# JacksonCampolattaro/spectrogram-rs

Hardware: AMD Instinct MI355X
Metric: STFT frames/sec (4096-pt, hop 256) (higher is better)
Workload: dtype f32

## Files before the change

spectrogram_rs_amd/csrc/stft4096_real.hip:

```cpp
#include <cmath>
#include <type_traits>

#include "stft4096_wg.hpp"

namespace sgx {

namespace wgr {

using wg::kBufComplex;
using wg::kLdsBytes;
using wg::kLdsBytesRender;
using wg::kM;
using wg::kS1;
using wg::kS2;
using wg::kW;
using wg::lds_barrier;
using wg::lds_read_alone;
using wg::lds_cfloat2;
using wg::lds_ptr;
using wg::pcm_rsrc;
using wg::u32x2;
using wg::u32x4;

typedef float f2v __attribute__((ext_vector_type(2)));
__device__ __forceinline__ float cl_fma(float a, float c, float u) { return fmaf(a, c, u); }
__device__ __forceinline__ f2v cl_fma(f2v a, float c, f2v u) { return __builtin_elementwise_fma(a, f2v{c, c}, u); }

#include "fft_codelets.inc"

using wg::Params;

__device__ __forceinline__ float2 cmulf(float2 a, float2 b)
{
    return make_float2(fmaf(a.x, b.x, -(a.y * b.y)), fmaf(a.x, b.y, a.y * b.x));
}

__device__ __forceinline__ __amdgpu_buffer_rsrc_t out_rsrc(char *base, long long byte, bool present)
{
    const uint32_t lo = __builtin_amdgcn_readfirstlane((uint32_t)byte);
    const uint32_t hi = __builtin_amdgcn_readfirstlane((uint32_t)((unsigned long long)byte >> 32));
    const int records = __builtin_amdgcn_readfirstlane(present ? 0x7fffffff : 0);
    return __builtin_amdgcn_make_buffer_rsrc(base + (long long)(((unsigned long long)hi << 32) | lo), 0, records, 0x00020000);
}

__device__ __forceinline__ void fft8_half_zero(const float (&zr)[4], const float (&zi)[4], float (&yr)[8], float (&yi)[8])
{
    constexpr float kH = 0.70710678118654752440f;
    auto fft4 = [](float a0r, float a0i, float a1r, float a1i, float a2r, float a2i, float a3r, float a3i, float *outr, float *outi) {
        const float s0r = a0r + a2r, s0i = a0i + a2i, s1r = a0r - a2r, s1i = a0i - a2i;
        const float s2r = a1r + a3r, s2i = a1i + a3i, s3r = a1r - a3r, s3i = a1i - a3i;
        outr[0] = s0r + s2r; outi[0] = s0i + s2i;
        outr[4] = s0r - s2r; outi[4] = s0i - s2i;
        outr[2] = s1r + s3i; outi[2] = s1i - s3r;
        outr[6] = s1r - s3i; outi[6] = s1i + s3r;
    };
    fft4(zr[0], zi[0], zr[1], zi[1], zr[2], zi[2], zr[3], zi[3], yr, yi);
    const float y1r = (zr[1] + zi[1]) * kH, y1i = (zi[1] - zr[1]) * kH;
    const float y3r = (zi[3] - zr[3]) * kH, y3i = -(zr[3] + zi[3]) * kH;
    fft4(zr[0], zi[0], y1r, y1i, zi[2], -zr[2], y3r, y3i, yr + 1, yi + 1);
}

constexpr int kRowsF32 = 0, kRowsF16 = 1, kPixels = 2;
constexpr int kBands = 3;
constexpr int kPeak = 5;
constexpr int kRowsC64 = 4;

#ifndef SGX_K1R_INTERLEAVE
#define SGX_K1R_INTERLEAVE 1
#endif
#ifndef SGX_SAMPLE_EARLY
#define SGX_SAMPLE_EARLY 1
#endif
#ifndef SGX_ADDTID_R
#define SGX_ADDTID_R 1
#endif
constexpr int kPlaneIm = 4480;
constexpr int kBufComplexTR = kPlaneIm;
static_assert(kBufComplexTR >= kBufComplex && 16 * 280 <= kPlaneIm, "the planes hold both images");
constexpr size_t kLdsBytesR = (size_t)(kBufComplexTR + 256) * sizeof(float2);
constexpr size_t kLdsBytesRenderR = kLdsBytesR + 256 * sizeof(uint2);
static_assert(4 * kLdsBytesRenderR <= 160 * 1024, "four workgroups per CU");
template <int STRIDE>
__device__ __forceinline__ void addtid_rows(float2 a, float2 b, uint32_t m0_wave, int ra, int rb)
{
    asm volatile("s_mov_b32 m0, %4\n\t"
                 "s_nop 0\n\t"
                 "ds_write_addtid_b32 %0 offset:%5\n\t"
                 "ds_write_addtid_b32 %1 offset:%6\n\t"
                 "ds_write_addtid_b32 %2 offset:%7\n\t"
                 "ds_write_addtid_b32 %3 offset:%8"
                 :
                 : "v"(a.x), "v"(a.y), "v"(b.x), "v"(b.y), "s"(m0_wave), "i"(4 * STRIDE * ra), "i"(4 * STRIDE * ra + 4 * kPlaneIm), "i"(4 * STRIDE * rb), "i"(4 * STRIDE * rb + 4 * kPlaneIm)
                 : "memory");
}
__device__ __forceinline__ void read_planes(const float4 *rd4, float (&xr)[16], float (&xi)[16])
{
#pragma unroll
    for (int c = 0; c < 4; ++c) {
        const float4 r = rd4[c], i = rd4[c + kPlaneIm / 4];
        xr[4 * c] = r.x; xr[4 * c + 1] = r.y; xr[4 * c + 2] = r.z; xr[4 * c + 3] = r.w;
        xi[4 * c] = i.x; xi[4 * c + 1] = i.y; xi[4 * c + 2] = i.z; xi[4 * c + 3] = i.w;
    }
}
__device__ __forceinline__ float lane_xor8(float v) { return __int_as_float(__builtin_amdgcn_mov_dpp(__float_as_int(v), 0x128, 0xf, 0xf, true)); }

#if SGX_STAMPS
__device__ unsigned long long g_phase_cycles_r[24];
#define SGX_STAMP(i) { const unsigned long long now_ = __builtin_readcyclecounter(); st_acc[i] += now_ - st_last; st_last = now_; }
#else
#define SGX_STAMP(i)
#endif

template <int MODE, int PIX, bool SLIDE>
__global__ void __launch_bounds__(256, 4) stft4096_real_kernel(Params p)
{
    extern __shared__ __attribute__((aligned(16))) unsigned char smem_raw[];
    float2 *buf = reinterpret_cast<float2 *>(smem_raw);
    constexpr bool TR = SLIDE && SGX_ADDTID_R;
    float2 *tw2 = buf + (TR ? kBufComplexTR : kBufComplex);
    uint2 *pal = reinterpret_cast<uint2 *>(tw2 + 256);
    constexpr bool F16 = MODE == kRowsF16;
    constexpr bool C64 = MODE == kRowsC64;
    constexpr bool FUSED = MODE == kPixels || MODE == kBands || MODE == kPeak;

    const int tid = threadIdx.x;
    const int t_p1 = TR ? (tid >> 4) + 16 * (tid & 15) : tid;
    float *plane = reinterpret_cast<float *>(smem_raw);
    const uint32_t m0_wave = __builtin_amdgcn_readfirstlane((uint32_t)(tid >> 6) * 272u);
    const float4 *rd4_1 = reinterpret_cast<const float4 *>(plane + 272 * (tid >> 4) + 68 * ((tid & 15) >> 2) + 16 * (tid & 3));
    const float4 *rd4_2 = reinterpret_cast<const float4 *>(plane + 280 * ((tid & 127) >> 3) + 68 * ((8 * (tid >> 7) + (tid & 7)) >> 2) + 16 * (tid & 3));
    tw2[tid] = p.tw2[tid];
    uint32_t row_words[4] = {0u, 0u, 0u, 0u};
    if (FUSED) {
        if (MODE == kPixels) pal[tid] = make_uint2(__float_as_uint(tid < 255 ? p.lut_thr[tid] : __builtin_nanf("")), *reinterpret_cast<const uint32_t *>(&p.lut_rgba[tid]));
#pragma unroll
        for (int i = 0; i < 4; ++i)
            if ((uint32_t)tid + 256u * i < p.R) row_words[i] = p.rows[tid + 256 * i];
    }

    float win[8];
#pragma unroll
    for (int a = 0; a < 4; ++a) {
        win[2 * a] = p.window[2 * t_p1 + 512 * a] * (1.0f / 2048.0f);
        win[2 * a + 1] = p.window[2 * t_p1 + 512 * a + 1] * (1.0f / 2048.0f);
    }
    float2 tw1[8];
#pragma unroll
    for (int q = 1; q < 8; ++q) tw1[q] = p.tw1[q * 256 + t_p1];
    const int F = tid >> 7, u = tid & 127;
    float2 twu[8];
#pragma unroll
    for (int q = 0; q < 8; ++q) twu[q] = p.twu[q * 128 + u];
    const int g2 = tid >> 4, t0_2 = tid & 15;
    const int cbase2 = (g2 >> 3) * 128 + (g2 & 7);
    __syncthreads();

    const unsigned long long job_begin = (unsigned long long)blockIdx.x * p.jobs_per_block;
    unsigned long long job_end = job_begin + p.jobs_per_block;
    if (job_end > p.n_jobs) job_end = p.n_jobs;
    if (job_begin >= job_end) return;

    auto samples_from = [&](unsigned long long first) {
        const unsigned long long left = first < p.stream_samples ? (p.stream_samples - first) * 4 : 0;
        const unsigned long long addr = (unsigned long long)(p.pcm + (first < p.stream_samples ? first : 0));
        const uint32_t lo = __builtin_amdgcn_readfirstlane((uint32_t)addr), hi = __builtin_amdgcn_readfirstlane((uint32_t)(addr >> 32));
        const int records = __builtin_amdgcn_readfirstlane((int)(left < 0x7fffffffull ? left : 0x7fffffffull));
        return __builtin_amdgcn_make_buffer_rsrc(reinterpret_cast<void *>(((unsigned long long)hi << 32) | lo), 0, records, 0x00020000);
    };
    auto columns_from = [&](unsigned long long col0) { return samples_from(2 * col0); };
    auto column = [&](__amdgpu_buffer_rsrc_t r, int byte_offset) {
        const u32x2 v = __builtin_amdgcn_raw_buffer_load_b64(r, t_p1 * 8, byte_offset, 0);
        return make_float2(__uint_as_float(v.x), __uint_as_float(v.y));
    };
    float2 R[8];
    float2 L;
    auto load_pair = [&](unsigned long long fa_) {
        const __amdgpu_buffer_rsrc_t r0 = samples_from(fa_ * p.H), r1 = samples_from((fa_ + 1) * p.H);
#pragma unroll
        for (int a = 0; a < 4; ++a) { R[2 * a] = column(r0, 2048 * a); R[2 * a + 1] = column(r1, 2048 * a); }
    };
    {
        const __amdgpu_buffer_rsrc_t r0 = columns_from(128 * (p.first_frame + 2 * job_begin));
        if (SLIDE) {
#pragma unroll
            for (int j = 0; j < 8; ++j) R[j] = column(r0, 1024 * j);
            L = column(r0, 9216);
        } else {
            load_pair(p.first_frame + 2 * job_begin);
            L = R[7];
        }
#pragma unroll
        for (int j = 0; j < 8; ++j) asm volatile("" ::"v"(R[j].x), "v"(R[j].y));
        asm volatile("" ::"v"(L.x), "v"(L.y));
#pragma unroll
        for (int q = 1; q < 8; ++q) asm volatile("" ::"v"(tw1[q].x), "v"(tw1[q].y));
#pragma unroll
        for (int q = 0; q < 8; ++q) asm volatile("" ::"v"(twu[q].x), "v"(twu[q].y), "v"(win[q]));
    }
    float2 *xch = buf + 2304;

    char *out = reinterpret_cast<char *>(p.mags);
    constexpr int kBin = C64 ? 16 : (F16 ? 4 : 8);
#if SGX_STAMPS
    unsigned long long st_acc[20] = {0, 0, 0, 0, 0, 0, 0, 0, 0, 0, 0, 0, 0, 0, 0, 0, 0, 0, 0, 0};
    unsigned long long st_last = __builtin_readcyclecounter();
#endif
    for (unsigned long long job = job_begin; job < job_end; ++job) {
        SGX_STAMP(19)
        const unsigned long long fa = p.first_frame + 2 * job;
        const unsigned long long la = 2 * job, lb = la + 1;
        const bool have_b = lb < p.n_frames;

        float yr[8], yi[8];
        {
            float zr[4], zi[4];
#pragma unroll
            for (int a = 0; a < 4; ++a) { zr[a] = R[2 * a].x * win[2 * a]; zi[a] = R[2 * a].y * win[2 * a + 1]; }
            fft8_half_zero(zr, zi, yr, yi);
        }
        float vr[8], vi[8];
        {
            float zr[4], zi[4];
#pragma unroll
            for (int a = 0; a < 4; ++a) { zr[a] = R[2 * a + 1].x * win[2 * a]; zi[a] = R[2 * a + 1].y * win[2 * a + 1]; }
            fft8_half_zero(zr, zi, vr, vi);
        }
        SGX_STAMP(0)
        lds_barrier();
        SGX_STAMP(1)
#pragma unroll
        for (int q = 0; q < 8; ++q) {
            const float2 ya = make_float2(yr[q], yi[q]), yb = make_float2(vr[q], vi[q]);
            if (TR) {
                addtid_rows<272>(q == 0 ? ya : cmulf(ya, tw1[q]), q == 0 ? yb : cmulf(yb, tw1[q]), m0_wave, q, 8 + q);
            } else {
                buf[q * kS1 + tid] = q == 0 ? ya : cmulf(ya, tw1[q]);
                buf[(8 + q) * kS1 + tid] = q == 0 ? yb : cmulf(yb, tw1[q]);
            }
        }
        __builtin_amdgcn_s_setprio(0);
        SGX_STAMP(2)
        lds_barrier();
        SGX_STAMP(3)

        float xr[16], xi[16];
        if (TR) {
            read_planes(rd4_1, xr, xi);
        } else {
#pragma unroll
            for (int t1 = 0; t1 < 16; ++t1) {
                const float2 v = buf[g2 * kS1 + t0_2 + 16 * t1];
                xr[t1] = v.x; xi[t1] = v.y;
            }
        }
        fft16(xr, xi);
        SGX_STAMP(4)
        lds_barrier();
        SGX_STAMP(5)
        if (TR) {
            lds_cfloat2 *tw2p = lds_ptr(tw2 + t0_2);
#pragma unroll
            for (int q2 = 0; q2 < 16; q2 += 2) {
                const int pa = FFT16_OUT[q2], pb = FFT16_OUT[q2 + 1];
                const float2 va = make_float2(xr[pa], xi[pa]), vb = make_float2(xr[pb], xi[pb]);
                addtid_rows<280>(q2 == 0 ? va : cmulf(va, lds_read_alone(tw2p, q2 * 16)), cmulf(vb, lds_read_alone(tw2p, (q2 + 1) * 16)), m0_wave, q2, q2 + 1);
            }
        } else {
#pragma unroll
            for (int q2 = 0; q2 < 16; ++q2) {
                const int pos = FFT16_OUT[q2];
                const float2 v = make_float2(xr[pos], xi[pos]);
                buf[t0_2 * kS2 + cbase2 + 8 * q2] = q2 == 0 ? v : cmulf(v, tw2[q2 * 16 + t0_2]);
            }
        }
        SGX_STAMP(6)
        lds_barrier();
        SGX_STAMP(7)

        if (TR) {
            read_planes(rd4_2, xr, xi);
        } else {
#pragma unroll
            for (int t0 = 0; t0 < 16; ++t0) {
                const float2 v = buf[t0 * kS2 + tid];
                xr[t0] = v.x; xi[t0] = v.y;
            }
        }
        fft16(xr, xi);

        float2 Ln = make_float2(0.0f, 0.0f);
        if (SLIDE && !FUSED) Ln = column(columns_from(128 * (fa + 2) + 1152), 0);
        if (!SLIDE) load_pair(fa + 2);

        if (FUSED) __builtin_amdgcn_s_setprio(1);
        else __builtin_amdgcn_s_setprio(3);
        SGX_STAMP(8)
        lds_barrier();
        SGX_STAMP(9)
#pragma unroll
        for (int j = 0; j < 8; ++j) {
            const int pos = FFT16_OUT[8 + j];
            buf[j * 256 + tid] = make_float2(xr[pos], xi[pos]);
        }
        if (SLIDE && !TR) {
            xch[tid].x = tid < 128 ? L.x : R[7].x;
            xch[tid].y = tid < 128 ? L.y : R[7].y;
        }
        SGX_STAMP(10)
        lds_barrier();
        SGX_STAMP(11)
        if (SLIDE) {
            const float2 Y = TR ? make_float2(lane_xor8((tid & 8) ? R[7].x : L.x), lane_xor8((tid & 8) ? R[7].y : L.y)) : xch[(tid + 128) & 255];
#pragma unroll
            for (int j = 0; j < 6; ++j) R[j] = R[j + 2];
            R[6] = Y;
            R[7] = L;
        }

        const int pcol = F * 128 + (u == 0 ? 256 : 128 - u);
        float m1[8], m2[8];
        constexpr bool kInterleave = (!FUSED && SLIDE && SGX_K1R_INTERLEAVE) || C64;
        const long long row = (long long)(F == 0 ? la : lb) * (long long)kM * kBin - kBin;
        const __amdgpu_buffer_rsrc_t r = out_rsrc(out, !FUSED ? row : 0, !FUSED && (F == 0 || have_b));
        const int l1 = kBin * u, l2 = kBin * (1152 - u);
        auto store_pair = [&](const int q3) {
            const float a = m1[q3], b = (q3 == 0 && u == 0) ? m1[0] : m2[q3];
            const int o1 = (q3 == 0 && u == 0) ? kBin * 1024 : l1;
            const int o2 = (q3 == 0 && u == 0) ? kBin * 128 : l2;
            const int s1 = kBin * 128 * q3, s2 = kBin * 128 * (7 - q3);
            if (F16) {
                const __half2 ha = __floats2half2_rn(a, a), hb = __floats2half2_rn(b, b);
                __builtin_amdgcn_raw_buffer_store_b32(*reinterpret_cast<const uint32_t *>(&ha), r, o1 + (s1 & 2047), s1 & ~2047, 0);
                __builtin_amdgcn_raw_buffer_store_b32(*reinterpret_cast<const uint32_t *>(&hb), r, o2 + (s2 & 2047), s2 & ~2047, 0);
            } else {
                __builtin_amdgcn_raw_buffer_store_b64(u32x2{__float_as_uint(a), __float_as_uint(a)}, r, o1 + (s1 & 2047), s1 & ~2047, 0);
                __builtin_amdgcn_raw_buffer_store_b64(u32x2{__float_as_uint(b), __float_as_uint(b)}, r, o2 + (s2 & 2047), s2 & ~2047, 0);
            }
        };
        float2 pvs[8];
        if (kInterleave) {
#pragma unroll
            for (int q3 = 0; q3 < 8; ++q3) pvs[q3] = buf[(7 - q3) * 256 + pcol];
        }
#pragma unroll
        for (int q3 = 0; q3 < 8; ++q3) {
            const int pos = FFT16_OUT[q3];
            float zr_ = xr[pos], zi_ = xi[pos];
            float2 pv = kInterleave ? pvs[q3] : buf[(7 - q3) * 256 + pcol];
            if (q3 == 0) {
                const float2 own = buf[F * 128];
                const int p8 = FFT16_OUT[8];
                zr_ = u == 0 ? xr[p8] : zr_; zi_ = u == 0 ? xi[p8] : zi_;
                pv.x = u == 0 ? own.x : pv.x; pv.y = u == 0 ? own.y : pv.y;
            }
            const float er = zr_ + pv.x, ei = zi_ - pv.y;
            const float orr = zi_ + pv.y, oi = pv.x - zr_;
            const float wr = fmaf(twu[q3].x, orr, -(twu[q3].y * oi)), wi = fmaf(twu[q3].x, oi, twu[q3].y * orr);
            const float ar = er + wr, ai = ei + wi, br = er - wr, bi = ei - wi;
            if constexpr (C64) {
                const bool self = q3 == 0 && u == 0;
                const float cr2 = self ? ar : br, ci2 = self ? ai : -bi;
                const int o1 = self ? kBin * 1024 : l1, o2 = self ? kBin * 128 : l2;
                const int s1 = kBin * 128 * q3, s2 = kBin * 128 * (7 - q3);
                __builtin_amdgcn_raw_buffer_store_b128(u32x4{__float_as_uint(ar), __float_as_uint(ai), __float_as_uint(ar), __float_as_uint(ai)}, r, o1 + s1, 0, 0);
                __builtin_amdgcn_raw_buffer_store_b128(u32x4{__float_as_uint(cr2), __float_as_uint(ci2), __float_as_uint(cr2), __float_as_uint(ci2)}, r, o2 + s2, 0, 0);
                __builtin_amdgcn_sched_barrier(0);
                continue;
            }
            m1[q3] = __builtin_amdgcn_sqrtf(fmaf(ar, ar, ai * ai));
            m2[q3] = __builtin_amdgcn_sqrtf(fmaf(br, br, bi * bi));
            if (kInterleave) {
                store_pair(q3);
                __builtin_amdgcn_sched_barrier(0);
            }
        }

        if (!FUSED) {
            if (!kInterleave) {
#pragma unroll
                for (int q3 = 0; q3 < 8; ++q3) store_pair(q3);
            }
        } else {
            float2 *mpair = buf;
            float2 *vbuf = mpair + wg::kColSlots;
            float *mcol = reinterpret_cast<float *>(buf) + F;
            lds_barrier();
            SGX_STAMP(13)
            constexpr bool kEarlyWords = SGX_SAMPLE_EARLY && PIX != wg::kPixGeneric;
            wg::SampleWords sw;
            const __amdgpu_buffer_rsrc_t rt_words = wg::pcm_rsrc(reinterpret_cast<const float *>(p.samples));
            int tid_w = tid;
            asm volatile("" : "+v"(tid_w));
#pragma unroll
            for (int q3 = 0; q3 < 8; ++q3) {
                const bool self = q3 == 0 && u == 0;
                const int k1 = self ? 1024 : u + 128 * q3, k2 = self ? 1024 : 2048 - u - 128 * q3;
                mcol[2 * k1] = m1[q3];
                mcol[2 * k2] = self ? m1[0] : m2[q3];
                if (q3 == 0 && u == 1) {
                    mcol[0] = m1[0];
                    mcol[2 * (kM + 1)] = mcol[2 * (kM + 2)] = m2[0];
                }
                if (kEarlyWords) {
                    sw.se[q3] = wg::sample_word(rt_words, p, (uint32_t)tid_w + 256u * q3);
                    __builtin_amdgcn_sched_barrier(0);
                }
            }
            if (kEarlyWords) sw.se[8] = wg::sample_word(rt_words, p, (uint32_t)tid_w + 2048u);
            static_assert(wg::kSampleSteps == 9 && wg::kSampleEarly == 9, "one word per column-write step and one behind them");
            SGX_STAMP(14)
            lds_barrier();
            SGX_STAMP(15)
            if (kEarlyWords) wg::sample_pass_with<PIX>(p, mpair, vbuf, tid, sw);
            else wg::sample_pass<PIX>(p, mpair, vbuf, tid);
            [[maybe_unused]] wg::PeakDst peak_a{}, peak_b{};
            [[maybe_unused]] wg::PeakOld<true> peak_old{};
            if constexpr (MODE == kPeak) {
                peak_a = wg::peak_dst(p, la);
                peak_b = have_b ? wg::peak_dst_next(p, peak_a, lb) : peak_a;
                peak_old = wg::peak_prefetch<true>(p, peak_a, tid);
            }
            if (SLIDE) L = column(columns_from(128 * (fa + 2) + 1152), 0);
            SGX_STAMP(16)
            lds_barrier();
            SGX_STAMP(17)
            __builtin_amdgcn_s_setprio(3);
            if constexpr (MODE == kPeak) {
                wg::row_pass_peak<true>(p, row_words, vbuf, peak_a, peak_b, peak_old, have_b, tid);
            } else if constexpr (MODE == kBands) {
                float2 *bands = reinterpret_cast<float2 *>(p.rgba);
                wg::row_pass_bands<true>(p, row_words, vbuf, bands + la * (size_t)p.R, bands + lb * (size_t)p.R, true, have_b, tid);
            } else {
                uchar4 *rgba = reinterpret_cast<uchar4 *>(p.rgba);
                wg::row_pass<true, PIX>(p, row_words, vbuf, rgba + la * (size_t)p.R, rgba + lb * (size_t)p.R, true, have_b, pal, tid);
            }
        }
        if (SLIDE && !FUSED) {
            asm volatile("" : "+v"(Ln.x), "+v"(Ln.y));
            L = Ln;
        }
        SGX_STAMP(18)
    }
#if SGX_STAMPS
    if ((tid & 63) == 0) {
#pragma unroll
        for (int i = 0; i < 20; ++i) atomicAdd(&g_phase_cycles_r[i], st_acc[i]);
        atomicAdd(&g_phase_cycles_r[20], (unsigned long long)(job_end - job_begin));
    }
#endif
}

struct RealTables {
    float2 *d_tw1 = nullptr, *d_tw2 = nullptr, *d_twu = nullptr;
};

}

#if SGX_STAMPS
extern "C" __attribute__((visibility("default"))) int sgx_debug_phase_cycles_r(unsigned long long *h_out, int reset)
{
    hipError_t e = hipMemcpyFromSymbol(h_out, HIP_SYMBOL(wgr::g_phase_cycles_r), sizeof(unsigned long long) * 24);
    if (e == hipSuccess && reset) {
        unsigned long long zero[24] = {0};
        e = hipMemcpyToSymbol(HIP_SYMBOL(wgr::g_phase_cycles_r), zero, sizeof(zero));
    }
    return e == hipSuccess ? 0 : -1;
}
#endif

hipError_t real4096_init(sgx_ctx *c, void **out)
{
    using namespace wgr;
    (void)c;
    auto *t = new RealTables();
    auto unit = [](unsigned long long e, unsigned long long n) {
        e %= n;
        if (e == 0) return make_float2(1.0f, 0.0f);
        if (4 * e == n) return make_float2(0.0f, -1.0f);
        if (2 * e == n) return make_float2(-1.0f, 0.0f);
        if (4 * e == 3 * n) return make_float2(0.0f, 1.0f);
        const double ang = -2.0 * M_PI * (double)e / (double)n;
        return make_float2((float)cos(ang), (float)sin(ang));
    };
    std::vector<float2> tw1(8 * 256), tw2(256), twu(8 * 128);
    for (int q = 0; q < 8; ++q)
        for (int tt = 0; tt < 256; ++tt) tw1[q * 256 + tt] = unit((unsigned long long)tt * q, 2048);
    for (int q = 0; q < 16; ++q)
        for (int t0 = 0; t0 < 16; ++t0) tw2[q * 16 + t0] = unit((unsigned long long)t0 * q, 256);
    for (int q3 = 0; q3 < 8; ++q3)
        for (int uu = 0; uu < 128; ++uu) twu[q3 * 128 + uu] = unit((unsigned long long)(uu + 128 * q3), 4096);
    twu[0] = unit(1024, 4096);
    auto up = [](float2 **dst, const std::vector<float2> &v) {
        hipError_t e = hipMalloc(reinterpret_cast<void **>(dst), v.size() * sizeof(float2));
        if (e == hipSuccess) e = hipMemcpy(*dst, v.data(), v.size() * sizeof(float2), hipMemcpyHostToDevice);
        return e;
    };
    hipError_t e = up(&t->d_tw1, tw1);
    if (e == hipSuccess) e = up(&t->d_tw2, tw2);
    if (e == hipSuccess) e = up(&t->d_twu, twu);
    if (e != hipSuccess) {
        real4096_destroy(t);
        return e;
    }
    *out = t;
    return hipSuccess;
}

void real4096_destroy(void *tables)
{
    auto *t = static_cast<wgr::RealTables *>(tables);
    if (!t) return;
    if (t->d_tw1) (void)hipFree(t->d_tw1);
    if (t->d_tw2) (void)hipFree(t->d_tw2);
    if (t->d_twu) (void)hipFree(t->d_twu);
    delete t;
}

bool real4096_serves(const sgx_ctx *c, const float *d_pcm, uint32_t channels)
{
    (void)d_pcm;
    return channels == 1 && c->d_real && c->W == (uint32_t)wgr::kW;
}

namespace wg {

hipError_t launch_real4096(const sgx_ctx *c, const void *real_tables, Params p, bool out_f16, bool render, bool bands, bool out_c64, bool peak)
{
    using namespace wgr;
    if (p.n_frames == 0) return hipSuccess;
    const auto *t = static_cast<const RealTables *>(real_tables);
    p.tw1 = t->d_tw1;
    p.tw2 = t->d_tw2;
    p.twu = t->d_twu;
    p.stream_samples = p.total_frames ? (p.total_frames - 1) * (unsigned long long)c->H + (unsigned long long)kW : 0;
    p.n_jobs = (p.n_frames + 1) / 2;
    unsigned long long blocks = (unsigned long long)c->n_cu * 4;
    unsigned long long per = (p.n_jobs + blocks - 1) / blocks;
    if (per < 1) per = 1;
    if (peak) {
        per = peak_align_run(per, 2, p.peak_group);
        p.peak_run = 2 * per;
    }
    blocks = (p.n_jobs + per - 1) / per;
    p.jobs_per_block = per;
    const dim3 grid((unsigned)blocks), block(256);
    auto launch = [&](auto slide_c) {
        constexpr bool S_ = decltype(slide_c)::value;
        constexpr size_t lds_rows = (S_ && SGX_ADDTID_R) ? kLdsBytesR : kLdsBytes, lds_render = (S_ && SGX_ADDTID_R) ? kLdsBytesRenderR : kLdsBytesRender;
        if (render && bands && peak) {
            if (p.interp == SGX_INTERP_COSINE) hipLaunchKernelGGL((stft4096_real_kernel<kPeak, kPixPeakCosine, S_>), grid, block, lds_rows, c->stream, p);
            else hipLaunchKernelGGL((stft4096_real_kernel<kPeak, kPixPeakCubic, S_>), grid, block, lds_rows, c->stream, p);
        } else if (render && bands) {
            if (p.interp == SGX_INTERP_COSINE) hipLaunchKernelGGL((stft4096_real_kernel<kBands, kPixBandsCosine, S_>), grid, block, lds_rows, c->stream, p);
            else hipLaunchKernelGGL((stft4096_real_kernel<kBands, kPixBandsCubic, S_>), grid, block, lds_rows, c->stream, p);
        } else if (render) {
            if (!p.seed_pm1) hipLaunchKernelGGL((stft4096_real_kernel<kPixels, kPixGeneric, S_>), grid, block, lds_render, c->stream, p);
            else if (p.interp == SGX_INTERP_COSINE) hipLaunchKernelGGL((stft4096_real_kernel<kPixels, kPixCosine, S_>), grid, block, lds_render, c->stream, p);
            else hipLaunchKernelGGL((stft4096_real_kernel<kPixels, kPixCubic, S_>), grid, block, lds_render, c->stream, p);
        } else if (out_c64) {
            hipLaunchKernelGGL((stft4096_real_kernel<kRowsC64, kPixNone, S_>), grid, block, lds_rows, c->stream, p);
        } else if (out_f16) {
            hipLaunchKernelGGL((stft4096_real_kernel<kRowsF16, kPixNone, S_>), grid, block, lds_rows, c->stream, p);
        } else {
            hipLaunchKernelGGL((stft4096_real_kernel<kRowsF32, kPixNone, S_>), grid, block, lds_rows, c->stream, p);
        }
    };
    if (c->H == 256) launch(std::true_type{});
    else launch(std::false_type{});
    const hipError_t e = hipGetLastError();
    return e == hipSuccess && peak ? launch_peak_combine(c, p, blocks) : e;
}

}

}
```

Baseline: 296.0 million.

## Defer row stores into next job and keep second-stage twiddles in registers

```diff
diff --git a/spectrogram_rs_amd/csrc/stft4096_real.hip b/spectrogram_rs_amd/csrc/stft4096_real.hip
--- a/spectrogram_rs_amd/csrc/stft4096_real.hip
+++ b/spectrogram_rs_amd/csrc/stft4096_real.hip
@@ -80,6 +80,25 @@
 constexpr size_t kLdsBytesR = (size_t)(kBufComplexTR + 256) * sizeof(float2);
 constexpr size_t kLdsBytesRenderR = kLdsBytesR + 256 * sizeof(uint2);
 static_assert(4 * kLdsBytesRenderR <= 160 * 1024, "four workgroups per CU");
+#ifndef SGX_K1R_HOLD
+#define SGX_K1R_HOLD 7
+#endif
+#ifndef SGX_K1R_PACE
+#define SGX_K1R_PACE 1
+#endif
+#ifndef SGX_K1R_PRIO
+#define SGX_K1R_PRIO 9
+#endif
+#ifndef SGX_K1R_PA
+#define SGX_K1R_PA 1
+#define SGX_K1R_PB 1
+#define SGX_K1R_PC 0
+#define SGX_K1R_PD 0
+#endif
+constexpr bool hold_level(int mode, bool slide, int bit) { return mode == 0  && slide && SGX_ADDTID_R && (SGX_K1R_HOLD & 1) && (SGX_K1R_HOLD & bit); }
+constexpr int kPartnerComplex = 8 * 256;
+constexpr size_t kLdsBytesHold = (SGX_K1R_HOLD & 4) ? (size_t)(kBufComplexTR + kPartnerComplex) * sizeof(float2) : kLdsBytesR;
+static_assert(3 * ((kLdsBytesHold + 1279) / 1280 * 1280) <= 160 * 1024, "three workgroups per CU (LDS is allocated in pieces of 1 280 B)");
 template <int STRIDE>
 __device__ __forceinline__ void addtid_rows(float2 a, float2 b, uint32_t m0_wave, int ra, int rb)
 {
@@ -112,7 +131,7 @@
 #endif
 
 template <int MODE, int PIX, bool SLIDE>
-__global__ void __launch_bounds__(256, 4) stft4096_real_kernel(Params p)
+__global__ void __launch_bounds__(256, hold_level(MODE, SLIDE, 1) ? 3 : 4) stft4096_real_kernel(Params p)
 {
     extern __shared__ __attribute__((aligned(16))) unsigned char smem_raw[];
     float2 *buf = reinterpret_cast<float2 *>(smem_raw);
@@ -122,6 +141,12 @@
     constexpr bool F16 = MODE == kRowsF16;
     constexpr bool C64 = MODE == kRowsC64;
     constexpr bool FUSED = MODE == kPixels || MODE == kBands || MODE == kPeak;
+    constexpr bool P9 = SGX_K1R_PRIO == 9 && MODE == kRowsF32 && SLIDE;
+    constexpr bool WG3 = hold_level(MODE, SLIDE, 1);
+    constexpr bool HOLD = hold_level(MODE, SLIDE, 2);
+    constexpr bool OWN = hold_level(MODE, SLIDE, 4);
+    static_assert(kRowsF32 == 0, "hold_level names the mode by its value");
+    float2 *part = OWN ? tw2 : buf;
 
     const int tid = threadIdx.x;
     const int t_p1 = TR ? (tid >> 4) + 16 * (tid & 15) : tid;
@@ -129,7 +154,12 @@
     const uint32_t m0_wave = __builtin_amdgcn_readfirstlane((uint32_t)(tid >> 6) * 272u);
     const float4 *rd4_1 = reinterpret_cast<const float4 *>(plane + 272 * (tid >> 4) + 68 * ((tid & 15) >> 2) + 16 * (tid & 3));
     const float4 *rd4_2 = reinterpret_cast<const float4 *>(plane + 280 * ((tid & 127) >> 3) + 68 * ((8 * (tid >> 7) + (tid & 7)) >> 2) + 16 * (tid & 3));
-    tw2[tid] = p.tw2[tid];
+    if (!OWN) tw2[tid] = p.tw2[tid];
+    float2 tw2r[16];
+    if (OWN) {
+#pragma unroll
+        for (int q2 = 1; q2 < 16; ++q2) tw2r[q2] = p.tw2[q2 * 16 + (tid & 15)];
+    }
     uint32_t row_words[4] = {0u, 0u, 0u, 0u};
     if (FUSED) {
         if (MODE == kPixels) pal[tid] = make_uint2(__float_as_uint(tid < 255 ? p.lut_thr[tid] : __builtin_nanf("")), *reinterpret_cast<const uint32_t *>(&p.lut_rgba[tid]));
@@ -196,11 +226,55 @@
         for (int q = 1; q < 8; ++q) asm volatile("" ::"v"(tw1[q].x), "v"(tw1[q].y));
 #pragma unroll
         for (int q = 0; q < 8; ++q) asm volatile("" ::"v"(twu[q].x), "v"(twu[q].y), "v"(win[q]));
+        if (OWN) {
+#pragma unroll
+            for (int q2 = 1; q2 < 16; ++q2) asm volatile("" ::"v"(tw2r[q2].x), "v"(tw2r[q2].y));
+        }
     }
     float2 *xch = buf + 2304;
 
     char *out = reinterpret_cast<char *>(p.mags);
     constexpr int kBin = C64 ? 16 : (F16 ? 4 : 8);
+
+    float m1[8], m2[8];
+    __amdgpu_buffer_rsrc_t r_held = out_rsrc(out, 0, false);
+    if (HOLD) {
+#pragma unroll
+        for (int q = 0; q < 8; ++q) m1[q] = m2[q] = 0.0f;
+    }
+    const int u_out = tid & 127;
+    auto store_one = [&](const int q3) {
+        if (HOLD) {
+            const bool self = q3 == 0 && u_out == 0;
+            const float a = m1[q3], b = self ? m1[0] : m2[q3];
+            const int o1 = self ? 8 * 1024 : 8 * u_out, o2 = self ? 8 * 128 : 8 * (1152 - u_out);
+            const int s1 = 1024 * q3, s2 = 1024 * (7 - q3);
+            __builtin_amdgcn_sched_barrier(0);
+            __builtin_amdgcn_raw_buffer_store_b64(u32x2{__float_as_uint(a), __float_as_uint(a)}, r_held, o1 + (s1 & 2047), s1 & ~2047, 0);
+            __builtin_amdgcn_raw_buffer_store_b64(u32x2{__float_as_uint(b), __float_as_uint(b)}, r_held, o2 + (s2 & 2047), s2 & ~2047, 0);
+            __builtin_amdgcn_sched_barrier(0);
+        }
+    };
+    auto store_held = [&](const int pos) {
+        if (SGX_K1R_PACE == 0 || pos < 0) {
+            if (pos >= 0) store_one(pos);
+            else {
+#pragma unroll
+                for (int q3 = 0; q3 < 8; ++q3) store_one(q3);
+            }
+        } else if (SGX_K1R_PACE == 1) {
+            if (pos == 0) {
+#pragma unroll
+                for (int q3 = 0; q3 < 8; ++q3) store_one(q3);
+            }
+        } else {
+            if (pos == 1 || pos == 2 || pos == 4 || pos == 7) {
+                const int g = pos == 1 ? 0 : pos == 2 ? 1 : pos == 4 ? 2 : 3;
+                store_one(2 * g);
+                store_one(2 * g + 1);
+            }
+        }
+    };
 #if SGX_STAMPS
     unsigned long long st_acc[20] = {0, 0, 0, 0, 0, 0, 0, 0, 0, 0, 0, 0, 0, 0, 0, 0, 0, 0, 0, 0};
     unsigned long long st_last = __builtin_readcyclecounter();
@@ -210,6 +284,7 @@
         const unsigned long long fa = p.first_frame + 2 * job;
         const unsigned long long la = 2 * job, lb = la + 1;
         const bool have_b = lb < p.n_frames;
+        if (P9) __builtin_amdgcn_s_setprio(SGX_K1R_PA);
 
         float yr[8], yi[8];
         {
@@ -218,6 +293,7 @@
             for (int a = 0; a < 4; ++a) { zr[a] = R[2 * a].x * win[2 * a]; zi[a] = R[2 * a].y * win[2 * a + 1]; }
             fft8_half_zero(zr, zi, yr, yi);
         }
+        store_held(0);
         float vr[8], vi[8];
         {
             float zr[4], zi[4];
@@ -225,8 +301,9 @@
             for (int a = 0; a < 4; ++a) { zr[a] = R[2 * a + 1].x * win[2 * a]; zi[a] = R[2 * a + 1].y * win[2 * a + 1]; }
             fft8_half_zero(zr, zi, vr, vi);
         }
+        store_held(1);
         SGX_STAMP(0)
-        lds_barrier();
+        if (!OWN) lds_barrier();
         SGX_STAMP(1)
 #pragma unroll
         for (int q = 0; q < 8; ++q) {
@@ -237,13 +314,16 @@
                 buf[q * kS1 + tid] = q == 0 ? ya : cmulf(ya, tw1[q]);
                 buf[(8 + q) * kS1 + tid] = q == 0 ? yb : cmulf(yb, tw1[q]);
             }
-        }
-        __builtin_amdgcn_s_setprio(0);
+            if (q == 3) store_held(2);
+        }
+        if ((!WG3 || SGX_K1R_PRIO == 1) && !P9) __builtin_amdgcn_s_setprio(0);
+        if (P9) __builtin_amdgcn_s_setprio(SGX_K1R_PB);
         SGX_STAMP(2)
         lds_barrier();
         SGX_STAMP(3)
 
         float xr[16], xi[16];
+        store_held(3);
         if (TR) {
             read_planes(rd4_1, xr, xi);
         } else {
@@ -254,6 +334,7 @@
             }
         }
         fft16(xr, xi);
+        store_held(4);
         SGX_STAMP(4)
         lds_barrier();
         SGX_STAMP(5)
@@ -263,7 +344,9 @@
             for (int q2 = 0; q2 < 16; q2 += 2) {
                 const int pa = FFT16_OUT[q2], pb = FFT16_OUT[q2 + 1];
                 const float2 va = make_float2(xr[pa], xi[pa]), vb = make_float2(xr[pb], xi[pb]);
-                addtid_rows<280>(q2 == 0 ? va : cmulf(va, lds_read_alone(tw2p, q2 * 16)), cmulf(vb, lds_read_alone(tw2p, (q2 + 1) * 16)), m0_wave, q2, q2 + 1);
+                if (OWN) addtid_rows<280>(q2 == 0 ? va : cmulf(va, tw2r[q2]), cmulf(vb, tw2r[q2 + 1]), m0_wave, q2, q2 + 1);
+                else addtid_rows<280>(q2 == 0 ? va : cmulf(va, lds_read_alone(tw2p, q2 * 16)), cmulf(vb, lds_read_alone(tw2p, (q2 + 1) * 16)), m0_wave, q2, q2 + 1);
+                if (q2 == 6) store_held(5);
             }
         } else {
 #pragma unroll
@@ -277,6 +360,8 @@
         lds_barrier();
         SGX_STAMP(7)
 
+        if (P9) __builtin_amdgcn_s_setprio(SGX_K1R_PC);
+        store_held(6);
         if (TR) {
             read_planes(rd4_2, xr, xi);
         } else {
@@ -287,20 +372,22 @@
             }
         }
         fft16(xr, xi);
+        store_held(7);
+        if (P9) __builtin_amdgcn_s_setprio(SGX_K1R_PD);
 
         float2 Ln = make_float2(0.0f, 0.0f);
-        if (SLIDE && !FUSED) Ln = column(columns_from(128 * (fa + 2) + 1152), 0);
+        if (SLIDE && !FUSED && !HOLD) Ln = column(columns_from(128 * (fa + 2) + 1152), 0);
         if (!SLIDE) load_pair(fa + 2);
 
         if (FUSED) __builtin_amdgcn_s_setprio(1);
-        else __builtin_amdgcn_s_setprio(3);
+        else if ((!WG3 || SGX_K1R_PRIO == 1) && !P9) __builtin_amdgcn_s_setprio(3);
         SGX_STAMP(8)
-        lds_barrier();
+        if (!OWN) lds_barrier();
         SGX_STAMP(9)
 #pragma unroll
         for (int j = 0; j < 8; ++j) {
             const int pos = FFT16_OUT[8 + j];
-            buf[j * 256 + tid] = make_float2(xr[pos], xi[pos]);
+            part[j * 256 + tid] = make_float2(xr[pos], xi[pos]);
         }
         if (SLIDE && !TR) {
             xch[tid].x = tid < 128 ? L.x : R[7].x;
@@ -315,10 +402,10 @@
             for (int j = 0; j < 6; ++j) R[j] = R[j + 2];
             R[6] = Y;
             R[7] = L;
+            if (HOLD) L = column(columns_from(128 * (fa + 2) + 1152), 0);
         }
 
         const int pcol = F * 128 + (u == 0 ? 256 : 128 - u);
-        float m1[8], m2[8];
         constexpr bool kInterleave = (!FUSED && SLIDE && SGX_K1R_INTERLEAVE) || C64;
         const long long row = (long long)(F == 0 ? la : lb) * (long long)kM * kBin - kBin;
         const __amdgpu_buffer_rsrc_t r = out_rsrc(out, !FUSED ? row : 0, !FUSED && (F == 0 || have_b));
@@ -340,15 +427,15 @@
         float2 pvs[8];
         if (kInterleave) {
 #pragma unroll
-            for (int q3 = 0; q3 < 8; ++q3) pvs[q3] = buf[(7 - q3) * 256 + pcol];
+            for (int q3 = 0; q3 < 8; ++q3) pvs[q3] = part[(q3 == 0 && OWN && u == 0) ? F * 128 : (7 - q3) * 256 + pcol];
         }
 #pragma unroll
         for (int q3 = 0; q3 < 8; ++q3) {
             const int pos = FFT16_OUT[q3];
             float zr_ = xr[pos], zi_ = xi[pos];
-            float2 pv = kInterleave ? pvs[q3] : buf[(7 - q3) * 256 + pcol];
+            float2 pv = kInterleave ? pvs[q3] : part[(7 - q3) * 256 + pcol];
             if (q3 == 0) {
-                const float2 own = buf[F * 128];
+                const float2 own = part[F * 128];
                 const int p8 = FFT16_OUT[8];
                 zr_ = u == 0 ? xr[p8] : zr_; zi_ = u == 0 ? xi[p8] : zi_;
                 pv.x = u == 0 ? own.x : pv.x; pv.y = u == 0 ? own.y : pv.y;
@@ -369,14 +456,15 @@
             }
             m1[q3] = __builtin_amdgcn_sqrtf(fmaf(ar, ar, ai * ai));
             m2[q3] = __builtin_amdgcn_sqrtf(fmaf(br, br, bi * bi));
-            if (kInterleave) {
+            if (kInterleave && !HOLD) {
                 store_pair(q3);
                 __builtin_amdgcn_sched_barrier(0);
             }
         }
+        if (HOLD) r_held = r;
 
         if (!FUSED) {
-            if (!kInterleave) {
+            if (!kInterleave && !HOLD) {
 #pragma unroll
                 for (int q3 = 0; q3 < 8; ++q3) store_pair(q3);
             }
@@ -435,11 +523,14 @@
                 wg::row_pass<true, PIX>(p, row_words, vbuf, rgba + la * (size_t)p.R, rgba + lb * (size_t)p.R, true, have_b, pal, tid);
             }
         }
-        if (SLIDE && !FUSED) {
+        if (SLIDE && !FUSED && !HOLD) {
             asm volatile("" : "+v"(Ln.x), "+v"(Ln.y));
             L = Ln;
         }
         SGX_STAMP(18)
+    }
+    if (HOLD) {
+        store_held(-1);
     }
 #if SGX_STAMPS
     if ((tid & 63) == 0) {
@@ -534,7 +625,8 @@
     p.twu = t->d_twu;
     p.stream_samples = p.total_frames ? (p.total_frames - 1) * (unsigned long long)c->H + (unsigned long long)kW : 0;
     p.n_jobs = (p.n_frames + 1) / 2;
-    unsigned long long blocks = (unsigned long long)c->n_cu * 4;
+    const bool three = hold_level(kRowsF32, true, 1) && c->H == 256 && !render && !out_c64 && !out_f16;
+    unsigned long long blocks = (unsigned long long)c->n_cu * (three ? 3 : 4);
     unsigned long long per = (p.n_jobs + blocks - 1) / blocks;
     if (per < 1) per = 1;
     if (peak) {
@@ -562,7 +654,7 @@
         } else if (out_f16) {
             hipLaunchKernelGGL((stft4096_real_kernel<kRowsF16, kPixNone, S_>), grid, block, lds_rows, c->stream, p);
         } else {
-            hipLaunchKernelGGL((stft4096_real_kernel<kRowsF32, kPixNone, S_>), grid, block, lds_rows, c->stream, p);
+            hipLaunchKernelGGL((stft4096_real_kernel<kRowsF32, kPixNone, S_>), grid, block, hold_level(kRowsF32, S_, 1) ? kLdsBytesHold : lds_rows, c->stream, p);
         }
     };
     if (c->H == 256) launch(std::true_type{});
```

After: 295.8 million (median of 2 runs). About the same (-0.1%).
